# blobcache/glfs

Measured on AMD Instinct MI355X. Metric: GiB/s hashed, device-resident 1 MiB chunks, bigblob write; 1/2/4/8 MI355X, higher is better.
Workload: dtype u32; 1 GPU; bigblob write 64 GiB/GPU @ 1024 KiB blocks, device-resident, ctext to HBM; blob_bytes=68719476736, block_size=1048576, blocks=65536, parallelism=disjoint block ranges x1

## Files before the change

### glfs_amd/csrc/one_classes.h

```cpp
#pragma once
#include <cstddef>
#include <cstdint>
#include <vector>

namespace glfsx {

enum OneClass : uint8_t { kOneSmall = 0, kOneMed = 1, kOneOpen = 2, kOneOpenSalted = 3 };
constexpr int kOneClasses = 4;

struct OneItem {
  bool open;
  bool salted;
  uint64_t len;
};

struct OneLayout {
  uint32_t count[kOneClasses] = {0, 0, 0, 0};
  uint32_t start[kOneClasses] = {0, 0, 0, 0};
  uint64_t max_len[kOneClasses] = {0, 0, 0, 0};
  uint64_t med_bytes = 0;
  std::vector<uint8_t> cls;
  std::vector<uint32_t> slot;
  std::vector<uint64_t> med_off;
};

inline uint64_t one_med_span(uint64_t len) { return (len + 255) & ~uint64_t(255); }

inline OneClass one_class(const OneItem &it, uint64_t small_max) {
  if (it.open) return it.salted ? kOneOpenSalted : kOneOpen;
  return it.len <= small_max ? kOneSmall : kOneMed;
}

inline OneLayout one_layout(const OneItem *items, size_t n, uint64_t small_max) {
  OneLayout L;
  L.cls.resize(n);
  L.slot.resize(n);
  L.med_off.assign(n, 0);
  for (size_t k = 0; k < n; ++k) {
    const OneClass c = one_class(items[k], small_max);
    L.cls[k] = c;
    ++L.count[c];
    if (items[k].len > L.max_len[c]) L.max_len[c] = items[k].len;
  }
  L.start[kOneSmall] = 0;
  L.start[kOneMed] = L.count[kOneSmall];
  L.start[kOneOpen] = 0;
  L.start[kOneOpenSalted] = L.count[kOneOpen];
  uint32_t next[kOneClasses];
  for (int c = 0; c < kOneClasses; ++c) next[c] = L.start[c];
  for (size_t k = 0; k < n; ++k) {
    const uint8_t c = L.cls[k];
    L.slot[k] = next[c]++;
    if (c == kOneMed) {
      L.med_off[k] = L.med_bytes;
      L.med_bytes += one_med_span(items[k].len);
    }
  }
  return L;
}

}
```

### glfs_amd/csrc/one_kernels.h

```cpp


__device__ __forceinline__ uint32_t img_g(uint32_t g) { return g ^ ((g >> 6) & 3u); }

__device__ __forceinline__ void one_chunks(uint32_t &cl, uint32_t &ch, uint32_t img,
                                           uint32_t len, uint32_t ctr0, bool root,
                                           uint32_t kq_lo, uint32_t kq_hi, uint32_t ivq,
                                           uint32_t base, uint32_t q, uint32_t quad,
                                           const uint32_t (&rel)[28]) {
  const uint32_t C = len ? (len + 1023) >> 10 : 1u;
  cl = kq_lo;
  ch = kq_hi;
  if (quad < C) {
    const uint32_t clen = min(len - min(len, quad << 10), 1024u);
    const uint32_t nb = clen ? (clen + 63) >> 6 : 1u;
    uint32_t addr[28];
#pragma unroll
    for (int k = 0; k < 28; ++k) {
      addr[k] = img + (quad << 10) + (rel[k] ^ (16u * (quad & 3u)));
      asm volatile("" : "+v"(addr[k]));
    }
    uint32_t m[4];
#pragma unroll
    for (int k = 0; k < 4; ++k) m[k] = *reinterpret_cast<lds_word>(addr[k]);
#pragma unroll
    for (int b = 0; b < 16; ++b) {
      if (uint32_t(b) < nb) {
        const uint32_t blen = min(clen - min(clen, 64u * b), 64u);
        uint32_t fl = base;
        if (b == 0) fl |= kChunkStart;
        if (uint32_t(b) + 1 == nb) {
          fl |= kChunkEnd;
          if (root && C == 1) fl |= kRoot;
        }
        const uint32_t dq = qsel(q, ctr0 + quad, 0u, blen, fl);
        uint32_t ab[28], nxt[4];
#pragma unroll
        for (int k = 0; k < 28; ++k) ab[k] = addr[k] + 64u * b;
        const uint32_t nb_off = uint32_t(b) + 1 < nb ? 64u * (b + 1) : 64u * b;
#pragma unroll
        for (int k = 0; k < 4; ++k) nxt[k] = addr[k] + nb_off;
        quad_compress_m<true>(cl, ch, ivq, dq, ab, m, nxt);
      }
    }
  }
}

__device__ __forceinline__ void one_tree(uint32_t &cl, uint32_t &ch, uint32_t count,
                                         bool root, uint32_t ts, uint32_t *passbuf,
                                         uint32_t kq_lo, uint32_t kq_hi, uint32_t ivq,
                                         uint32_t base, uint32_t q, uint32_t quad,
                                         const uint32_t (&rel)[28]) {
  while (count > 1) {
    const uint32_t half = count >> 1, odd = count & 1u;
    __syncthreads();
    if (quad < count) {
      if (odd && quad == count - 1) {
        passbuf[q] = cl;
        passbuf[4 + q] = ch;
      } else {
        const uint32_t sa = ts + ((quad >> 1) << 6) + ((quad & 1u) << 5) + 4u * q;
        *reinterpret_cast<__attribute__((address_space(3))) uint32_t *>(sa) = cl;
        *reinterpret_cast<__attribute__((address_space(3))) uint32_t *>(sa + 16u) = ch;
      }
    }
    __syncthreads();
    if (quad < half) {
      const uint32_t fl = base | kParent | ((root && count == 2) ? kRoot : 0u);
      cl = kq_lo;
      ch = kq_hi;
      const uint32_t dq = qsel(q, 0u, 0u, 64u, fl);
      uint32_t addr[28];
#pragma unroll
      for (int k = 0; k < 28; ++k) addr[k] = ts + (quad << 6) + rel[k];
      quad_compress(cl, ch, ivq, dq, addr);
    } else if (odd && quad == half) {
      cl = passbuf[q];
      ch = passbuf[4 + q];
    }
    count = half + odd;
  }
}

__device__ __forceinline__ void one_hash(uint32_t &cl, uint32_t &ch, uint32_t img,
                                         uint32_t ts, uint32_t *passbuf,
                                         uint32_t len, const uint32_t (&key)[8],
                                         uint32_t base, uint32_t q, uint32_t quad,
                                         const uint32_t (&rel)[28], uint32_t ctr0 = 0,
                                         bool root = true) {
  const uint32_t kq_lo = qsel(q, key[0], key[1], key[2], key[3]);
  const uint32_t kq_hi = qsel(q, key[4], key[5], key[6], key[7]);
  const uint32_t ivq = qsel(q, kIV[0], kIV[1], kIV[2], kIV[3]);
  one_chunks(cl, ch, img, len, ctr0, root, kq_lo, kq_hi, ivq, base, q, quad, rel);
  const uint32_t C = len ? (len + 1023) >> 10 : 1u;
  one_tree(cl, ch, C, root, ts, passbuf, kq_lo, kq_hi, ivq, base, q, quad, rel);
}

template <int LANES, int IT = 16>
__device__ __forceinline__ void one_stage(uint4 *img_u4, const uint8_t *src, uint32_t len,
                                          uint32_t present, uint8_t *dcopy) {
  const uint32_t padded = len ? (len + 63) & ~63u : 64u;
  const uint32_t have = min(len, present);
  uint4 v[IT];
#pragma unroll
  for (int i = 0; i < IT; ++i) {
    const uint32_t p = (threadIdx.x + uint32_t(i) * LANES) * 16u;
    v[i] = make_uint4(0, 0, 0, 0);
    if (p + 16u <= have) v[i] = *reinterpret_cast<const uint4 *>(src + p);
  }
#pragma unroll
  for (int i = 0; i < IT; ++i) {
    const uint32_t p = (threadIdx.x + uint32_t(i) * LANES) * 16u;
    if (p < padded) {
      if (p < have && p + 16u > have) {
        uint32_t w[4] = {0, 0, 0, 0};
        for (uint32_t k = 0; p + k < have; ++k) w[k >> 2] |= uint32_t(src[p + k]) << (8 * (k & 3));
        v[i] = make_uint4(w[0], w[1], w[2], w[3]);
      }
      img_u4[img_g(p >> 4)] = v[i];
      if (dcopy) *reinterpret_cast<uint4 *>(dcopy + p) = v[i];
    }
  }
}

template <int LANES>
__device__ __forceinline__ void one_xor(uint4 *img_u4, uint32_t len, const uint32_t (&dek)[8],
                                        uint32_t kb0) {
  const uint32_t nks = (len + 63) >> 6;
  for (uint32_t kb = threadIdx.x; kb < nks; kb += LANES) {
    uint32_t x[16];
    chacha_block<0>(x, dek, kb0 + kb);
    const uint32_t avail = min(len - kb * 64u, 64u);
    if (avail < 64) mask_tail(x, avail);
#pragma unroll
    for (int i = 0; i < 4; ++i) {
      uint4 v = img_u4[img_g(kb * 4 + i)];
      v.x ^= x[4 * i];
      v.y ^= x[4 * i + 1];
      v.z ^= x[4 * i + 2];
      v.w ^= x[4 * i + 3];
      img_u4[img_g(kb * 4 + i)] = v;
    }
  }
}

template <int LANES>
__device__ __forceinline__ void one_store(const uint4 *img_u4, uint8_t *dst, uint32_t len) {
  for (uint32_t p = threadIdx.x * 16u; p < len; p += LANES * 16u) {
    const uint4 v = img_u4[img_g(p >> 4)];
    if (p + 16u <= len) {
      *reinterpret_cast<uint4 *>(dst + p) = v;
    } else {
      const uint32_t w[4] = {v.x, v.y, v.z, v.w};
      for (uint32_t i = 0; p + i < len; ++i) dst[p + i] = uint8_t(w[i >> 2] >> (8 * (i & 3)));
    }
  }
}

template <class D>
__device__ __forceinline__ const D *one_desc(D *s, const D *g) {
  constexpr uint32_t kW = sizeof(D) / 4;
  static_assert(sizeof(D) % 4 == 0 && kW <= 64, "wave 0 stages the descriptor");
  if (threadIdx.x < kW)
    reinterpret_cast<uint32_t *>(s)[threadIdx.x] =
        reinterpret_cast<const uint32_t *>(g)[threadIdx.x];
  __syncthreads();
  return s;
}

template <class D>
__device__ __forceinline__ void one_signal(const D *dp) {
  asm volatile("s_waitcnt vmcnt(0)" ::: "memory");
  __syncthreads();
  if (threadIdx.x == 0 && dp->flag)
    __hip_atomic_store(dp->flag, dp->seq, __ATOMIC_RELEASE, __HIP_MEMORY_SCOPE_SYSTEM);
}

#if GLFSX_ONE_TIMING
__device__ unsigned long long g_one_t[16];
#define ONE_T(i)                                                                        \
  do {                                                                                  \
    if (blockIdx.x == 0 && threadIdx.x == 0)                                            \
      __hip_atomic_fetch_add(&g_one_t[i],                                               \
                             (unsigned long long)(__builtin_amdgcn_s_memrealtime() - t0), \
                             __ATOMIC_RELAXED, __HIP_MEMORY_SCOPE_AGENT);               \
  } while (0)
#else
#define ONE_T(i) \
  do {           \
  } while (0)
#endif

template <int QUADS, bool V>
__device__ __forceinline__ void one_run(const OneDesc *g) {
#if GLFSX_ONE_TIMING
  const uint64_t t0 = __builtin_amdgcn_s_memrealtime(), c0 = __builtin_amdgcn_s_memtime();
#endif
  __shared__ uint4 img_u4[QUADS * 64];
  __shared__ uint4 ts_u4[QUADS / 2 * 4];
  __shared__ uint32_t passbuf[8];
  __shared__ uint32_t s_dek[8];
  constexpr int kLanes = QUADS * 4;
  const OneDesc *dp;
  if constexpr (V) {
    dp = g;
  } else {
    __shared__ OneDesc s_desc;
    dp = one_desc(&s_desc, g + blockIdx.x);
  }
  const uint32_t len = dp->len;
  const uint32_t tid = threadIdx.x, q = tid & 3u, quad = tid >> 2;
  const uint32_t img = lds_offset(img_u4), ts = lds_offset(ts_u4);
  ONE_T(0);
  one_stage<kLanes>(img_u4, dp->src, len, dp->present, nullptr);
  uint32_t rel[28];
  quad_addrs(rel, 0u, q);
  __syncthreads();
  ONE_T(1);
  uint32_t key[8];
#pragma unroll
  for (int i = 0; i < 8; ++i) key[i] = dp->salt[i];
  uint32_t cl, ch;
#if GLFSX_ONE_TIMING
  {
    const uint32_t kq_lo = qsel(q, key[0], key[1], key[2], key[3]);
    const uint32_t kq_hi = qsel(q, key[4], key[5], key[6], key[7]);
    const uint32_t ivq = qsel(q, kIV[0], kIV[1], kIV[2], kIV[3]);
    one_chunks(cl, ch, img, len, 0u, true, kq_lo, kq_hi, ivq, kKeyed, q, quad, rel);
    ONE_T(6);
    one_tree(cl, ch, len ? (len + 1023) >> 10 : 1u, true, ts, passbuf, kq_lo, kq_hi, ivq,
             kKeyed, q, quad, rel);
  }
#else
  one_hash(cl, ch, img, ts, passbuf, len, key, kKeyed, q, quad, rel);
#endif
  if (quad == 0) {
    s_dek[q] = cl;
    s_dek[4 + q] = ch;
  }
  __syncthreads();
  ONE_T(2);
  uint32_t dek[8];
#pragma unroll
  for (int i = 0; i < 8; ++i) dek[i] = s_dek[i];
  one_xor<kLanes>(img_u4, len, dek, 0u);
  __syncthreads();
  ONE_T(3);
  if (dp->ctext) one_store<kLanes>(img_u4, dp->ctext, len);
  uint32_t ckey[8];
#pragma unroll
  for (int i = 0; i < 8; ++i) ckey[i] = dp->cid_key[i];
#if GLFSX_ONE_TIMING
  {
    const uint32_t cb = dp->cid_keyed ? kKeyed : 0u;
    const uint32_t kq_lo = qsel(q, ckey[0], ckey[1], ckey[2], ckey[3]);
    const uint32_t kq_hi = qsel(q, ckey[4], ckey[5], ckey[6], ckey[7]);
    const uint32_t ivq = qsel(q, kIV[0], kIV[1], kIV[2], kIV[3]);
    one_chunks(cl, ch, img, len, 0u, true, kq_lo, kq_hi, ivq, cb, q, quad, rel);
    ONE_T(7);
    one_tree(cl, ch, len ? (len + 1023) >> 10 : 1u, true, ts, passbuf, kq_lo, kq_hi, ivq, cb,
             q, quad, rel);
  }
#else
  one_hash(cl, ch, img, ts, passbuf, len, ckey, dp->cid_keyed ? kKeyed : 0u, q, quad, rel);
#endif
  if (quad == 0) {
    uint32_t *r = reinterpret_cast<uint32_t *>(dp->ref);
    r[q] = cl;
    r[4 + q] = ch;
    r[8 + q] = dek[q];
    r[12 + q] = dek[4 + q];
  }
  ONE_T(4);
  one_signal(dp);
  ONE_T(5);
#if GLFSX_ONE_TIMING
  if (blockIdx.x == 0 && threadIdx.x == 0) {
    const uint64_t c1 = __builtin_amdgcn_s_memtime(), t1 = __builtin_amdgcn_s_memrealtime();
    __hip_atomic_fetch_add(&g_one_t[13], (unsigned long long)(c1 - c0), __ATOMIC_RELAXED,
                           __HIP_MEMORY_SCOPE_AGENT);
    __hip_atomic_fetch_add(&g_one_t[14], (unsigned long long)(t1 - t0), __ATOMIC_RELAXED,
                           __HIP_MEMORY_SCOPE_AGENT);
    __hip_atomic_fetch_add(&g_one_t[15], 1ull, __ATOMIC_RELAXED, __HIP_MEMORY_SCOPE_AGENT);
  }
#endif
}

template <int QUADS>
__global__ __launch_bounds__(QUADS * 4) void k_one(const OneDesc *descs) {
  one_run<QUADS, false>(descs);
}

template <int QUADS>
__global__ __launch_bounds__(QUADS * 4) void k_one_v(const OneDesc d) {
  one_run<QUADS, true>(&d);
}

__device__ __forceinline__ void med_publish_merge(uint32_t &cl, uint32_t &ch, const OneDesc *dp,
                                                  uint32_t sidx, uint32_t W, uint32_t ts,
                                                  uint32_t *passbuf, uint32_t *flag,
                                                  const uint32_t (&key)[8], uint32_t base,
                                                  uint32_t q, uint32_t quad,
                                                  const uint32_t (&rel)[28], bool *last) {
  const uint32_t tid = threadIdx.x;
  if (quad == 0) {
    __hip_atomic_store(dp->cvs + sidx * 8 + q, cl, __ATOMIC_RELAXED, __HIP_MEMORY_SCOPE_AGENT);
    __hip_atomic_store(dp->cvs + sidx * 8 + 4 + q, ch, __ATOMIC_RELAXED,
                       __HIP_MEMORY_SCOPE_AGENT);
  }
  *last = arrive_last(dp->cnt, W, tid, flag);
  if (!*last) return;
// ... 130 lines not shown
```

### glfs_amd/csrc/post_kernels.hip

```cpp
#include "kernels.h"

#include <algorithm>
#include <atomic>
#include <cstdlib>
#include <cstring>
#include <mutex>
#include <type_traits>
#include <utility>

#include "device_common.h"
#include "launch_plan.h"
#include "stream_scratch.h"

namespace glfsx {
namespace {

#include "b3_arx.h"
#include "pass_kernels.h"
#include "quad_kernels.h"
#include "one_kernels.h"
#include "one_open_kernels.h"
#include "small_kernels.h"
#include "ragged_kernels.h"
#include "read_kernels.h"
#include "open_kernels.h"
#include "ragged_open_kernels.h"


std::atomic<uint32_t> g_latency_wgs{512}, g_split_target{2048u};
Knobs knobs() {
  return {g_split_target.load(std::memory_order_relaxed),
          g_latency_wgs.load(std::memory_order_relaxed)};
}

LaunchLog &g_launch_log = *new LaunchLog();
LaunchLog &g_aux_log = *new LaunchLog();

template <const auto &Gs, class F, size_t... I>
hipError_t with_g(uint32_t g, F &&f, std::index_sequence<I...>) {
  hipError_t e = hipErrorInvalidValue;
  (void)(... || (g == uint32_t(Gs[I]) && ((e = f(std::integral_constant<int, Gs[I]>{})), true)));
  return e;
}
template <const auto &Gs, class F>
hipError_t with_g(uint32_t g, F &&f) {
  return with_g<Gs>(g, f, std::make_index_sequence<std::size(Gs)>{});
}

template <int G, bool CHACHA, bool ALIGNED, int A>
bool try_pass(const LaunchRec &r, const KArgs &a, hipStream_t s) {
  if constexpr (pass_form_ok(G, CHACHA, ALIGNED, A)) {
    if (r.chacha == CHACHA && r.aligned == ALIGNED && r.form == A) {
      hipLaunchKernelGGL((k_pass<G, CHACHA, ALIGNED, A>), dim3(r.grid), dim3(256), 0, s, a);
      return true;
    }
  }
  return false;
}
template <int G, bool CHACHA>
bool try_pass_g(const LaunchRec &r, const KArgs &a, hipStream_t s) {
  return try_pass<G, CHACHA, true, 0>(r, a, s) || try_pass<G, CHACHA, true, 1>(r, a, s) ||
         try_pass<G, CHACHA, true, 2>(r, a, s) || try_pass<G, CHACHA, false, 2>(r, a, s);
}

// ... 422 lines not shown
  for (int i = 0; i < 3; ++i) totals[i] = __atomic_load_n(tot + i, __ATOMIC_RELAXED);
  if (totals[0] == 0) return hipSuccess;
  e = get(0, 4 * size_t(cv_words) * (totals[0] + totals[1]));
  a.gcv = a.cvs + cv_words * totals[0];
  return e;
}

template <bool CHACHA>
static hipError_t launch_rag_pass(RArgs a, const uint64_t tot[3], hipStream_t s) {
  a.total = tot[0];
  const GridForm p = rag_chunk_plan(tot[0], knobs().latency_wgs);
  if (p.form == 0)
    hipLaunchKernelGGL((k_rag_chunk<CHACHA, 0>), dim3(p.grid), dim3(256), 0, s, a);
  else
    hipLaunchKernelGGL((k_rag_chunk<CHACHA, 2>), dim3(p.grid), dim3(256), 0, s, a);
  hipError_t e = hipGetLastError();
  auto merge = [&](auto k, uint64_t total) {
    a.total = total;
    hipLaunchKernelGGL(k, dim3(capped_grid(total, 1u << 20)), dim3(256), 0, s, a);
    return hipGetLastError();
  };
  if (e == hipSuccess && tot[1]) e = merge(k_rag_merge_a, tot[1]);
  if (e == hipSuccess && tot[2]) e = merge(k_rag_merge_b, tot[2]);
  return e;
}

hipError_t launch_post_ragged(const RaggedJob &job, hipStream_t s) {
  if (job.n == 0) return hipSuccess;
  if (job.hi > kMaxRaggedLen) return hipErrorInvalidValue;
  RArgs a{};
  a.src = job.src;
  a.ctext = job.ctext;
  a.offs = job.offs;
  a.lens = job.lens;
  a.n = job.n;
  a.lo = job.lo;
  a.hi = job.hi;
  a.refs = job.refs;
  uint64_t totals[3];
  hipError_t e = rag_plan<false>(a, &ScratchSlot::rag, 8, nullptr, 0u, totals, s);
  if (e != hipSuccess || totals[0] == 0) return e;
  for (int i = 0; i < 8; ++i) a.key[i] = job.salt[i];
  a.base = kKeyed;
  a.out_off = 32;
  e = launch_rag_pass<false>(a, totals, s);
  if (e != hipSuccess) return e;
  for (int i = 0; i < 8; ++i) a.key[i] = job.cid_key[i];
  a.base = job.cid_keyed ? kKeyed : 0u;
  a.out_off = 0;
  return launch_rag_pass<true>(a, totals, s);
}

#if GLFSX_ONE_TIMING
extern "C" int glfsx_debug_one_timing(int reset, uint64_t out[16]) {
  if (hipMemcpyFromSymbol(out, HIP_SYMBOL(g_one_t), 16 * sizeof(uint64_t), 0,
                          hipMemcpyDeviceToHost) != hipSuccess)
    return -1;
  if (!reset) return 0;
  const unsigned long long z[16] = {};
  return hipMemcpyToSymbol(HIP_SYMBOL(g_one_t), z, sizeof z, 0, hipMemcpyHostToDevice) ==
                 hipSuccess ? 0 : -1;
}
#endif

size_t pass_log(int reset, uint32_t *out, size_t cap) {
  if (!g_launch_log.on()) g_launch_log.enable();
  return g_launch_log.read(reset != 0, out, cap);
}

size_t aux_log(int reset, uint32_t *out, size_t cap) {
  if (!g_aux_log.on()) g_aux_log.enable();
  return g_aux_log.read(reset != 0, out, cap);
}

hipError_t clock_probe(int reset, uint64_t out[2]) {
  g_clk_on.store(true, std::memory_order_relaxed);
  unsigned long long v[2] = {0, 0};
  hipError_t e = hipMemcpyFromSymbol(v, HIP_SYMBOL(g_clk), sizeof v, 0, hipMemcpyDeviceToHost);
  if (e != hipSuccess) return e;
  if (out) {
    out[0] = v[0];
    out[1] = v[1];
  }
  if (!reset) return hipSuccess;
  const unsigned long long z[2] = {0, 0};
  return hipMemcpyToSymbol(HIP_SYMBOL(g_clk), z, sizeof z, 0, hipMemcpyHostToDevice);
}

#if GLFSX_WGTIME
hipError_t debug_wgtime(uint64_t *out) {
  return hipMemcpyFromSymbol(out, HIP_SYMBOL(g_wgtime), sizeof(g_wgtime), 0,
                             hipMemcpyDeviceToHost);
}
#endif

template <class K, class A>
static hipError_t med_launch(K dek, K cid, uint32_t n, uint64_t len, const A &a, hipStream_t s) {
  if (len > kMaxMedLen || len <= kMaxOneLen) return hipErrorInvalidValue;
  const uint32_t wmax = uint32_t((len + 65535) >> 16);
  hipLaunchKernelGGL(dek, dim3(n * wmax), dim3(256), 0, s, a, wmax);
  hipError_t e = hipGetLastError();
  if (e != hipSuccess) return e;
  hipLaunchKernelGGL(cid, dim3(n * wmax), dim3(256), 0, s, a, wmax);
  return hipGetLastError();
}
hipError_t launch_med(const OneDesc *descs, uint32_t n, uint64_t max_len, hipStream_t s) {
  return n ? med_launch(k_med_dek, k_med_cid, n, max_len, descs, s) : hipSuccess;
}
hipError_t launch_med_v(const OneDesc &d, hipStream_t s) {
  return med_launch(k_med_dek_v, k_med_cid_v, 1, d.len, d, s);
}

template <class K, class A>
static hipError_t one_launch(K k16, K k64, uint32_t n, uint64_t len, const A &a, hipStream_t s) {
  if (len > kMaxOneLen) return hipErrorInvalidValue;
  if (len <= 16 * 1024)
    hipLaunchKernelGGL(k16, dim3(n), dim3(64), 0, s, a);
  else
    hipLaunchKernelGGL(k64, dim3(n), dim3(256), 0, s, a);
  return hipGetLastError();
}
hipError_t launch_one(const OneDesc *descs, uint32_t n, uint64_t max_len, hipStream_t s) {
  return n ? one_launch(k_one<16>, k_one<64>, n, max_len, descs, s) : hipSuccess;
}
hipError_t launch_one_v(const OneDesc &d, hipStream_t s) {
  return one_launch(k_one_v<16>, k_one_v<64>, 1, d.len, d, s);
}

template <class K, class A>
static hipError_t one_open_launch(K k16s, K k64s, K k16, K k64, uint32_t n, uint64_t len,
                                  bool salted, const A &a, hipStream_t s) {
  if (len > kMaxOneLen) return hipErrorInvalidValue;
  const bool small = len <= 16 * 1024;
  const K k = salted ? (small ? k16s : k64s) : (small ? k16 : k64);
  hipLaunchKernelGGL(k, dim3(n), dim3((small ? 16 : 64) * (salted ? 8 : 4)), 0, s, a);
  return hipGetLastError();
}
hipError_t launch_one_open(const OneOpenDesc *descs, uint32_t n, uint64_t max_len, bool salted,
                           hipStream_t s) {
  if (n == 0) return hipSuccess;
  return one_open_launch(k_one_open<16, true>, k_one_open<64, true>, k_one_open<16, false>,
                         k_one_open<64, false>, n, max_len, salted, descs, s);
}
hipError_t launch_one_open_v(const OneOpenDesc &d, bool salted, hipStream_t s) {
  return one_open_launch(k_one_open_v<16, true>, k_one_open_v<64, true>, k_one_open_v<16, false>,
                         k_one_open_v<64, false>, 1, d.len, salted, d, s);
}

hipError_t launch_decrypt(const uint8_t *ctext, uint8_t *ptext, uint64_t n, uint64_t bs,
                          uint64_t last_len, const uint8_t *refs, hipStream_t s) {
  return decrypt_with(ctext, ptext, n, bs, last_len, refs, knobs().latency_wgs, s);
}

hipError_t launch_chacha_xor(const uint32_t k[8], const uint8_t *src,
                             uint8_t *dst, uint64_t n, hipStream_t s) {
  if (n == 0) return hipSuccess;
  KArgs a{};
  a.src = src;
  a.ctext = dst;
  a.msg_len = n;
  for (int i = 0; i < 8; ++i) a.key[i] = k[i];
  const uint32_t grid = capped_grid((((n + 63) >> 6) + 255) / 256, 65536);
  hipLaunchKernelGGL(k_chacha_xor, dim3(grid), dim3(256), 0, s, a);
  return hipGetLastError();
}


static std::atomic<int> g_open_route{0};
int set_open_route(int route) {
// ... 131 lines not shown
```

### glfs_amd/csrc/quad_kernels.h

```cpp

#define QCOL0_ASM                                                               \
  "v_add_u32 %0, %1, %4\n"                                                      \
  "v_xor_b32 %3, %3, %0\n"                                                      \
  "v_alignbit_b32 %3, %3, %3, 16\n"                                             \
  "v_add_u32 %2, %2, %3\n"                                                      \
  "v_xor_b32 %1, %1, %2\n"                                                      \
  "v_alignbit_b32 %1, %1, %1, 12\n"
#define QCOL_ASM                                                                \
  "s_nop 0\n"                                                                   \
  "v_add_u32_dpp %0, %1, %4 quad_perm:[3,0,1,2] row_mask:0xf bank_mask:0xf\n"   \
  "v_xor_b32_dpp %3, %3, %0 quad_perm:[1,2,3,0] row_mask:0xf bank_mask:0xf\n"   \
  "v_alignbit_b32 %3, %3, %3, 16\n"                                             \
  "v_add_u32_dpp %2, %2, %3 quad_perm:[2,3,0,1] row_mask:0xf bank_mask:0xf\n"   \
  "v_xor_b32_dpp %1, %1, %2 quad_perm:[3,0,1,2] row_mask:0xf bank_mask:0xf\n"   \
  "v_alignbit_b32 %1, %1, %1, 12\n"
#define QREST_ASM                                                               \
  "v_add3_u32 %0, %0, %1, %5\n"                                                 \
  "v_xor_b32 %3, %3, %0\n"                                                      \
  "v_alignbit_b32 %3, %3, %3, 8\n"                                              \
  "v_add_u32 %2, %2, %3\n"                                                      \
  "v_xor_b32 %1, %1, %2\n"                                                      \
  "v_alignbit_b32 %1, %1, %1, 7\n"                                              \
  "v_add_u32 %4, %0, %6\n"                                                      \
  "s_nop 0\n"                                                                   \
  "v_add_u32_dpp %0, %1, %4 quad_perm:[1,2,3,0] row_mask:0xf bank_mask:0xf\n"   \
  "v_xor_b32_dpp %3, %3, %0 quad_perm:[3,0,1,2] row_mask:0xf bank_mask:0xf\n"   \
  "v_alignbit_b32 %3, %3, %3, 16\n"                                             \
  "v_add_u32_dpp %2, %2, %3 quad_perm:[2,3,0,1] row_mask:0xf bank_mask:0xf\n"   \
  "v_xor_b32_dpp %1, %1, %2 quad_perm:[1,2,3,0] row_mask:0xf bank_mask:0xf\n"   \
  "v_alignbit_b32 %1, %1, %1, 12\n"                                             \
  "v_add3_u32 %0, %0, %1, %7\n"                                                 \
  "v_xor_b32 %3, %3, %0\n"                                                      \
  "v_alignbit_b32 %3, %3, %3, 8\n"                                              \
  "v_add_u32 %2, %2, %3\n"                                                      \
  "v_xor_b32 %1, %1, %2\n"                                                      \
  "v_alignbit_b32 %1, %1, %1, 7\n"

typedef const __attribute__((address_space(3))) uint32_t *lds_word;
template <bool PF>
__device__ __forceinline__ void quad_compress_m(uint32_t &a, uint32_t &b, uint32_t c,
                                                uint32_t d, const uint32_t (&addr)[28],
                                                uint32_t (&m)[4], const uint32_t *nxt) {
#pragma unroll
  for (int r = 0; r < 7; ++r) {
    uint32_t n[4] = {0, 0, 0, 0};
    if (r < 6) {
#pragma unroll
      for (int k = 0; k < 4; ++k) n[k] = *reinterpret_cast<lds_word>(addr[4 * r + 4 + k]);
    } else if (PF) {
#pragma unroll
      for (int k = 0; k < 4; ++k) n[k] = *reinterpret_cast<lds_word>(nxt[k]);
    }
// ... 40 lines not shown
                              kSched.s[r][kk[k] + 4], kSched.s[r][kk[k] + 6]);
      addr[4 * r + k] = slot + 4u * (w ^ x);
    }
  }
}

__device__ __forceinline__ void tree_reduce_q(uint32_t *lds, uint32_t k, uint32_t t,
                              const uint32_t (&key)[8], uint32_t base, bool root,
                              uint32_t (&p)[8]) {
  const uint32_t q = t & 3u, quad = t >> 2;
  const uint32_t kq_lo = qsel(q, key[0], key[1], key[2], key[3]);
  const uint32_t kq_hi = qsel(q, key[4], key[5], key[6], key[7]);
  const uint32_t ivq = qsel(q, kIV[0], kIV[1], kIV[2], kIV[3]);
  uint32_t rel[28];
  quad_addrs(rel, lds_offset(lds), q);
  while (k > 1) {
    const uint32_t half = k >> 1, odd = k & 1u;
    const uint32_t fl = base | kParent | ((root && k == 2) ? kRoot : 0u);
    const uint32_t dq = qsel(q, 0u, 0u, 64u, fl);
    uint32_t rl[2] = {0, 0}, rh[2] = {0, 0};
#pragma unroll
    for (uint32_t r = 0; r < 2; ++r) {
      const uint32_t i = quad + 64u * r;
      if (i < half) {
        uint32_t addr[28];
#pragma unroll
        for (int x = 0; x < 28; ++x) addr[x] = rel[x] + 64u * i;
        uint32_t cl = kq_lo, ch = kq_hi;
        quad_compress(cl, ch, ivq, dq, addr);
        rl[r] = cl;
        rh[r] = ch;
      }
    }
    const uint32_t ov = (odd && t < 8) ? lds[(k - 1) * 8 + t] : 0u;
    __syncthreads();
#pragma unroll
    for (uint32_t r = 0; r < 2; ++r) {
      const uint32_t i = quad + 64u * r;
      if (i < half) {
        lds[i * 8 + q] = rl[r];
        lds[i * 8 + 4 + q] = rh[r];
      }
    }
    if (odd && t < 8) lds[half * 8 + t] = ov;
    __syncthreads();
    k = half + odd;
  }
  if (t == 0) {
#pragma unroll
    for (int i = 0; i < 8; ++i) p[i] = lds[i];
  }
}

template <int QPW>
__global__ __launch_bounds__(QPW * 4) void k_quad(KArgs a) {
  constexpr bool kTwo = QPW == 64;
  __shared__ uint4 slots[QPW * (kTwo ? 8 : 4)];
  __shared__ uint32_t passbuf[8];
  const uint32_t tid = threadIdx.x, q = tid & 3u, quad = tid >> 2;
  const uint64_t j = blockIdx.x >> a.split_log2;
  const uint32_t sidx = blockIdx.x & ((1u << a.split_log2) - 1u);
  const uint64_t len = (j + 1 == a.n) ? a.last_len : a.msg_len;
  constexpr uint64_t kSpan = uint64_t(QPW) << 10;
  const uint64_t c0b = uint64_t(sidx) * kSpan;
  if (sidx != 0 && c0b >= len) return;
  const bool whole = len <= kSpan;
  const uint64_t mylen = min(len - c0b, kSpan);
  const uint32_t cnt = mylen ? uint32_t((mylen + 1023) >> 10) : 1u;
  const uint8_t *msg = a.src + j * a.stride + c0b;
  const uint32_t slot = lds_offset(slots + quad * 4);
  const uint32_t kq_lo = qsel(q, a.key[0], a.key[1], a.key[2], a.key[3]);
  const uint32_t kq_hi = qsel(q, a.key[4], a.key[5], a.key[6], a.key[7]);
  const uint32_t ivq = qsel(q, kIV[0], kIV[1], kIV[2], kIV[3]);
  uint32_t addr[28];
  quad_addrs(addr, slot, q);
  uint32_t cl = kq_lo, ch = kq_hi;
  if (quad < cnt) {
    const uint64_t coff = uint64_t(quad) << 10;
    const uint32_t clen = uint32_t(min<uint64_t>(mylen - coff, 1024));
    const uint32_t nb = clen ? (clen + 63) >> 6 : 1u;
    const uint32_t ctr = sidx * uint32_t(QPW) + quad;
    const uint8_t *cp = msg + coff + 16u * q;
    uint4 blk[16];
#pragma unroll
    for (int b = 0; b < 16; ++b) {
      blk[b] = make_uint4(0, 0, 0, 0);
      const int32_t avail = int32_t(clen) - 64 * b - 16 * int32_t(q);
      if (avail >= 16) {
        blk[b] = *reinterpret_cast<const uint4 *>(cp + 64 * b);
      } else if (avail > 0) {
        uint32_t w[4] = {0, 0, 0, 0};
        for (int i = 0; i < avail; ++i) w[i >> 2] |= uint32_t(cp[64 * b + i]) << (8 * (i & 3));
        blk[b] = make_uint4(w[0], w[1], w[2], w[3]);
      }
    }
    const uint32_t x = kTwo ? 4u * ((quad >> 1) & 3u) : 0u;
    const uint32_t gq = 16u * (q ^ (x >> 2));
    constexpr uint32_t kB = kTwo ? QPW * 64u : 0u;
    uint32_t caddr[28];
    if constexpr (kTwo) {
      quad_addrs(caddr, slot, q, x);
#pragma unroll
      for (int k = 0; k < 28; ++k) asm volatile("" : "+v"(caddr[k]));
    }
    uint32_t m[4];
    if constexpr (kTwo) {
      *reinterpret_cast<lds_u32x4 *>(slot + gq) =
          u32x4{blk[0].x, blk[0].y, blk[0].z, blk[0].w};
      asm volatile("" ::: "memory");
#pragma unroll
      for (int k = 0; k < 4; ++k) m[k] = *reinterpret_cast<lds_word>(caddr[k]);
    }
#pragma unroll
    for (int b = 0; b < 16; ++b) {
      if (uint32_t(b) < nb) {
        const bool more = uint32_t(b) + 1 < nb;
        if constexpr (kTwo) {
          if (b + 1 < 16 && more)
            *reinterpret_cast<lds_u32x4 *>(slot + kB * ((b + 1) & 1) + gq) =
                u32x4{blk[(b + 1) & 15].x, blk[(b + 1) & 15].y, blk[(b + 1) & 15].z,
                      blk[(b + 1) & 15].w};
        } else {
          *reinterpret_cast<lds_u32x4 *>(slot + gq) =
              u32x4{blk[b].x, blk[b].y, blk[b].z, blk[b].w};
        }
        asm volatile("" ::: "memory");
        const uint32_t blen = min(clen - min(clen, 64u * b), 64u);
        uint32_t fl = a.base;
        if (b == 0) fl |= kChunkStart;
        if (uint32_t(b) + 1 == nb) {
          fl |= kChunkEnd;
          if (whole && cnt == 1) fl |= kRoot;
        }
        const uint32_t dq = qsel(q, ctr, 0u, blen, fl);
        if constexpr (kTwo) {
          uint32_t ab[28], nxt[4];
#pragma unroll
          for (int k = 0; k < 28; ++k) ab[k] = caddr[k] + kB * (b & 1);
          const uint32_t noff = more ? kB * ((b + 1) & 1) : kB * (b & 1);
#pragma unroll
          for (int k = 0; k < 4; ++k) nxt[k] = caddr[k] + noff;
          quad_compress_m<true>(cl, ch, ivq, dq, ab, m, nxt);
        } else {
          quad_compress(cl, ch, ivq, dq, addr);
        }
        asm volatile("" ::: "memory");
      }
    }
  }
  uint32_t count = cnt;
  while (count > 1) {
    const uint32_t half = count >> 1, odd = count & 1u;
    __syncthreads();
    if (quad < count) {
      if (odd && quad == count - 1) {
        passbuf[q] = cl;
        passbuf[4 + q] = ch;
      } else {
        uint32_t *ps = reinterpret_cast<uint32_t *>(slots + (quad >> 1) * 4);
        ps[(quad & 1u) * 8 + q] = cl;
        ps[(quad & 1u) * 8 + 4 + q] = ch;
      }
    }
    __syncthreads();
    if (quad < half) {
      const uint32_t fl = a.base | kParent | ((whole && count == 2) ? kRoot : 0u);
      cl = kq_lo;
      ch = kq_hi;
      const uint32_t dq = qsel(q, 0u, 0u, 64u, fl);
      quad_compress(cl, ch, ivq, dq, addr);
    } else if (odd && quad == half) {
      cl = passbuf[q];
      ch = passbuf[4 + q];
    }
    count = half + odd;
  }
  uint32_t *const out = reinterpret_cast<uint32_t *>(
      a.refs + (j / a.ref_bf) * a.ref_stride + (j % a.ref_bf) * 64 + a.out_off);
  if (whole) {
    if (quad == 0) {
      out[q] = cl;
      out[4 + q] = ch;
    }
    return;
  }
  const uint64_t wbase = j << a.split_log2;
  if (tid < 64) {
    uint32_t w[8];
#pragma unroll
    for (int k = 0; k < 4; ++k) {
      w[k] = __builtin_amdgcn_readlane(cl, k);
      w[4 + k] = __builtin_amdgcn_readlane(ch, k);
    }
    if (tid == 0) publish_cv(a.scratch + (wbase + sidx) * 8, w);
  }
  const uint32_t W = uint32_t((len + kSpan - 1) / kSpan);
  __shared__ uint32_t s_flag;
  if (!arrive_last(a.cnt + j, W, tid, &s_flag)) return;
  if (quad < W) {
    cl = load_cv_word(a.scratch + (wbase + quad) * 8 + q);
    ch = load_cv_word(a.scratch + (wbase + quad) * 8 + 4 + q);
  }
  count = W;
  while (count > 1) {
    const uint32_t half = count >> 1, odd = count & 1u;
    __syncthreads();
    if (quad < count) {
      if (odd && quad == count - 1) {
        passbuf[q] = cl;
        passbuf[4 + q] = ch;
      } else {
        uint32_t *ps = reinterpret_cast<uint32_t *>(slots + (quad >> 1) * 4);
        ps[(quad & 1u) * 8 + q] = cl;
        ps[(quad & 1u) * 8 + 4 + q] = ch;
      }
    }
    __syncthreads();
    if (quad < half) {
      const uint32_t fl = a.base | kParent | (count == 2 ? kRoot : 0u);
      cl = kq_lo;
      ch = kq_hi;
      const uint32_t dq = qsel(q, 0u, 0u, 64u, fl);
      quad_compress(cl, ch, ivq, dq, addr);
    } else if (odd && quad == half) {
      cl = passbuf[q];
      ch = passbuf[4 + q];
    }
    count = half + odd;
  }
  if (quad == 0) {
    out[q] = cl;
    out[4 + q] = ch;
    if (q == 0) a.cnt[j] = 0;
  }
}
```

Baseline: 968.6 GiB/s.

## Specialize full-chunk BLAKE3 path, add quad-parallel ChaCha XOR, tighten one-kernel threshold

Adds a FULL template specialization of the per-quad chunk compression. When a wave-wide ballot shows every chunk is a full 1 KiB, it uses precomputed flags and unconditional loads and skips the prefetch on the last block. It also adds a quad-cooperative ChaCha implementation using DPP lane permutes for the XOR stage, and lowers the single-wave launch threshold for the one-shot kernel from 16 KiB to 1 KiB. It further expands the debug timing counters. The goal is to remove per-block branch and flag arithmetic and to spread keystream work across more lanes, at the cost of larger code and more register pressure from the template duplication.

```diff
diff --git a/glfs_amd/csrc/one_classes.h b/glfs_amd/csrc/one_classes.h
--- a/glfs_amd/csrc/one_classes.h
+++ b/glfs_amd/csrc/one_classes.h
@@ -25,6 +25,8 @@
 };
 
 inline uint64_t one_med_span(uint64_t len) { return (len + 255) & ~uint64_t(255); }
+
+constexpr uint64_t kOneWaveMaxLen = 1024;
 
 inline OneClass one_class(const OneItem &it, uint64_t small_max) {
   if (it.open) return it.salted ? kOneOpenSalted : kOneOpen;
diff --git a/glfs_amd/csrc/one_kernels.h b/glfs_amd/csrc/one_kernels.h
--- a/glfs_amd/csrc/one_kernels.h
+++ b/glfs_amd/csrc/one_kernels.h
@@ -1,17 +1,28 @@
 
 
 __device__ __forceinline__ uint32_t img_g(uint32_t g) { return g ^ ((g >> 6) & 3u); }
+
+#if GLFSX_ONE_TIMING
+#define ONE_C_ARGS , uint64_t c0 = 0, int cslot = -1
+#define ONE_C_BLOCK(b) \
+  if (cslot >= 0) ONE_C(cslot + (b))
+#else
+#define ONE_C_ARGS
+#define ONE_C_BLOCK(b)
+#endif
 
 __device__ __forceinline__ void one_chunks(uint32_t &cl, uint32_t &ch, uint32_t img,
                                            uint32_t len, uint32_t ctr0, bool root,
                                            uint32_t kq_lo, uint32_t kq_hi, uint32_t ivq,
                                            uint32_t base, uint32_t q, uint32_t quad,
-                                           const uint32_t (&rel)[28]) {
+                                           const uint32_t (&rel)[28] ONE_C_ARGS) {
   const uint32_t C = len ? (len + 1023) >> 10 : 1u;
   cl = kq_lo;
   ch = kq_hi;
-  if (quad < C) {
-    const uint32_t clen = min(len - min(len, quad << 10), 1024u);
+  const bool mine = quad < C;
+  const uint32_t clen = mine ? min(len - min(len, quad << 10), 1024u) : 0u;
+  const bool full = __builtin_amdgcn_ballot_w64(mine && clen != 1024u) == 0;
+  if (mine) {
     const uint32_t nb = clen ? (clen + 63) >> 6 : 1u;
     uint32_t addr[28];
 #pragma unroll
@@ -22,6 +33,27 @@
     uint32_t m[4];
 #pragma unroll
     for (int k = 0; k < 4; ++k) m[k] = *reinterpret_cast<lds_word>(addr[k]);
+    if (full) {
+      const uint32_t lane3 = q == 3 ? ~0u : 0u;
+      const uint32_t dq = qsel(q, ctr0 + quad, 0u, 64u, base);
+      const uint32_t end = kChunkEnd | ((root && C == 1) ? kRoot : 0u);
+#pragma unroll
+      for (int b = 0; b < 16; ++b) {
+        uint32_t ab[28], nxt[4];
+#pragma unroll
+        for (int k = 0; k < 28; ++k) ab[k] = addr[k] + 64u * b;
+#pragma unroll
+        for (int k = 0; k < 4; ++k) nxt[k] = addr[k] + 64u * (b + 1);
+        if (b == 0)
+          quad_compress_m<true>(cl, ch, ivq, dq | (kChunkStart & lane3), ab, m, nxt);
+        else if (b < 15)
+          quad_compress_m<true>(cl, ch, ivq, dq, ab, m, nxt);
+        else
+          quad_compress_m<false>(cl, ch, ivq, dq | (end & lane3), ab, m, nullptr);
+        ONE_C_BLOCK(b);
+      }
+      return;
+    }
 #pragma unroll
     for (int b = 0; b < 16; ++b) {
       if (uint32_t(b) < nb) {
@@ -41,6 +73,7 @@
         for (int k = 0; k < 4; ++k) nxt[k] = addr[k] + nb_off;
         quad_compress_m<true>(cl, ch, ivq, dq, ab, m, nxt);
       }
+      ONE_C_BLOCK(b);
     }
   }
 }
@@ -122,10 +155,82 @@
   }
 }
 
+#define CQ_REST                                                                 \
+  "v_xor_b32 %3, %3, %0\n"                                                      \
+  "v_alignbit_b32 %3, %3, %3, 24\n"                                             \
+  "v_add_u32 %2, %2, %3\n"                                                      \
+  "v_xor_b32 %1, %1, %2\n"                                                      \
+  "v_alignbit_b32 %1, %1, %1, 25\n"
+#define CQ_COL0                                                                 \
+  "v_add_u32 %0, %0, %1\n"                                                      \
+  "v_xor_b32 %3, %3, %0\n"                                                      \
+  "v_alignbit_b32 %3, %3, %3, 16\n"                                             \
+  "v_add_u32 %2, %2, %3\n"                                                      \
+  "v_xor_b32 %1, %1, %2\n"                                                      \
+  "v_alignbit_b32 %1, %1, %1, 20\n"                                             \
+  "v_add_u32 %0, %0, %1\n" CQ_REST
+#define CQ_STEP(P1, P2, P3)                                                     \
+  "s_nop 1\n"                                                                   \
+  "v_add_u32_dpp %0, %1, %0 quad_perm:" P1 " row_mask:0xf bank_mask:0xf\n"      \
+  "v_xor_b32_dpp %3, %3, %0 quad_perm:" P3 " row_mask:0xf bank_mask:0xf\n"      \
+  "v_alignbit_b32 %3, %3, %3, 16\n"                                             \
+  "v_add_u32_dpp %2, %2, %3 quad_perm:" P2 " row_mask:0xf bank_mask:0xf\n"      \
+  "v_xor_b32_dpp %1, %1, %2 quad_perm:" P1 " row_mask:0xf bank_mask:0xf\n"      \
+  "v_alignbit_b32 %1, %1, %1, 20\n"                                             \
+  "v_add_u32 %0, %0, %1\n" CQ_REST
+#define CQ_DIAG CQ_STEP("[1,2,3,0]", "[2,3,0,1]", "[3,0,1,2]")
+#define CQ_COL CQ_STEP("[3,0,1,2]", "[2,3,0,1]", "[1,2,3,0]")
+
+__device__ __forceinline__ void chacha_quad(uint32_t &a, uint32_t &b, uint32_t &c, uint32_t &d,
+                                            const uint32_t (&k)[8], uint32_t ctr, uint32_t q) {
+  const uint32_t a0 = qsel(q, 0x61707865u, 0x3320646eu, 0x79622d32u, 0x6b206574u);
+  const uint32_t b0 = qsel(q, k[0], k[1], k[2], k[3]);
+  const uint32_t c0 = qsel(q, k[4], k[5], k[6], k[7]);
+  const uint32_t d0 = q == 0 ? ctr : 0u;
+  a = a0;
+  b = b0;
+  c = c0;
+  d = d0;
+  asm volatile(CQ_COL0 CQ_DIAG : "+v"(a), "+v"(b), "+v"(c), "+v"(d));
+#pragma unroll
+  for (int i = 1; i < 10; ++i)
+    asm volatile(CQ_COL CQ_DIAG : "+v"(a), "+v"(b), "+v"(c), "+v"(d));
+  asm volatile("v_add_u32 %0, %0, %4\n"
+               "v_add_u32_dpp %3, %3, %7 quad_perm:[1,2,3,0] row_mask:0xf bank_mask:0xf\n"
+               "v_add_u32_dpp %2, %2, %6 quad_perm:[2,3,0,1] row_mask:0xf bank_mask:0xf\n"
+               "v_add_u32_dpp %1, %1, %5 quad_perm:[3,0,1,2] row_mask:0xf bank_mask:0xf\n"
+               : "+v"(a), "+v"(b), "+v"(c), "+v"(d)
+               : "v"(a0), "v"(b0), "v"(c0), "v"(d0));
+}
+
 template <int LANES>
 __device__ __forceinline__ void one_xor(uint4 *img_u4, uint32_t len, const uint32_t (&dek)[8],
                                         uint32_t kb0) {
   const uint32_t nks = (len + 63) >> 6;
+  constexpr uint32_t kQuads = LANES / 4;
+  if ((nks + kQuads - 1) / kQuads <= 2u * ((nks + LANES - 1) / LANES)) {
+    const uint32_t q = threadIdx.x & 3u;
+    const uint32_t imgw = lds_offset(img_u4) + 4u * q;
+    for (uint32_t kb = threadIdx.x >> 2; kb < nks; kb += kQuads) {
+      uint32_t wa[4], v[4];
+#pragma unroll
+      for (int i = 0; i < 4; ++i) {
+        wa[i] = imgw + 16u * img_g(kb * 4 + i);
+        v[i] = *reinterpret_cast<lds_word>(wa[i]);
+      }
+      uint32_t x[4];
+      chacha_quad(x[0], x[1], x[2], x[3], dek, kb0 + kb, q);
+      const uint32_t avail = len - kb * 64u;
+#pragma unroll
+      for (int i = 0; i < 4; ++i) {
+        const uint32_t lo = 16u * i + 4u * q;
+        if (avail < lo + 4u)
+          x[i] &= avail <= lo ? 0u : (1u << (8u * (avail - lo))) - 1u;
+        *reinterpret_cast<__attribute__((address_space(3))) uint32_t *>(wa[i]) = v[i] ^ x[i];
+      }
+    }
+    return;
+  }
   for (uint32_t kb = threadIdx.x; kb < nks; kb += LANES) {
     uint32_t x[16];
     chacha_block<0>(x, dek, kb0 + kb);
@@ -176,13 +281,13 @@
 }
 
 #if GLFSX_ONE_TIMING
-__device__ unsigned long long g_one_t[16];
 #define ONE_T(i)                                                                        \
   do {                                                                                  \
     if (blockIdx.x == 0 && threadIdx.x == 0)                                            \
       __hip_atomic_fetch_add(&g_one_t[i],                                               \
                              (unsigned long long)(__builtin_amdgcn_s_memrealtime() - t0), \
                              __ATOMIC_RELAXED, __HIP_MEMORY_SCOPE_AGENT);               \
+    ONE_C(32 + (i));                                                                    \
   } while (0)
 #else
 #define ONE_T(i) \
@@ -225,7 +330,7 @@
     const uint32_t kq_lo = qsel(q, key[0], key[1], key[2], key[3]);
     const uint32_t kq_hi = qsel(q, key[4], key[5], key[6], key[7]);
     const uint32_t ivq = qsel(q, kIV[0], kIV[1], kIV[2], kIV[3]);
-    one_chunks(cl, ch, img, len, 0u, true, kq_lo, kq_hi, ivq, kKeyed, q, quad, rel);
+    one_chunks(cl, ch, img, len, 0u, true, kq_lo, kq_hi, ivq, kKeyed, q, quad, rel, c0, 16);
     ONE_T(6);
     one_tree(cl, ch, len ? (len + 1023) >> 10 : 1u, true, ts, passbuf, kq_lo, kq_hi, ivq,
              kKeyed, q, quad, rel);
@@ -246,6 +351,9 @@
   __syncthreads();
   ONE_T(3);
   if (dp->ctext) one_store<kLanes>(img_u4, dp->ctext, len);
+#if GLFSX_ONE_TIMING
+  ONE_C(56);
+#endif
   uint32_t ckey[8];
 #pragma unroll
   for (int i = 0; i < 8; ++i) ckey[i] = dp->cid_key[i];
@@ -255,7 +363,7 @@
     const uint32_t kq_lo = qsel(q, ckey[0], ckey[1], ckey[2], ckey[3]);
     const uint32_t kq_hi = qsel(q, ckey[4], ckey[5], ckey[6], ckey[7]);
     const uint32_t ivq = qsel(q, kIV[0], kIV[1], kIV[2], kIV[3]);
-    one_chunks(cl, ch, img, len, 0u, true, kq_lo, kq_hi, ivq, cb, q, quad, rel);
+    one_chunks(cl, ch, img, len, 0u, true, kq_lo, kq_hi, ivq, cb, q, quad, rel, c0, 40);
     ONE_T(7);
     one_tree(cl, ch, len ? (len + 1023) >> 10 : 1u, true, ts, passbuf, kq_lo, kq_hi, ivq, cb,
              q, quad, rel);
diff --git a/glfs_amd/csrc/post_kernels.hip b/glfs_amd/csrc/post_kernels.hip
--- a/glfs_amd/csrc/post_kernels.hip
+++ b/glfs_amd/csrc/post_kernels.hip
@@ -10,6 +10,7 @@
 
 #include "device_common.h"
 #include "launch_plan.h"
+#include "one_classes.h"
 #include "stream_scratch.h"
 
 namespace glfsx {
@@ -538,12 +539,12 @@
 }
 
 #if GLFSX_ONE_TIMING
-extern "C" int glfsx_debug_one_timing(int reset, uint64_t out[16]) {
-  if (hipMemcpyFromSymbol(out, HIP_SYMBOL(g_one_t), 16 * sizeof(uint64_t), 0,
+extern "C" int glfsx_debug_one_timing(int reset, uint64_t out[64]) {
+  if (hipMemcpyFromSymbol(out, HIP_SYMBOL(g_one_t), 64 * sizeof(uint64_t), 0,
                           hipMemcpyDeviceToHost) != hipSuccess)
     return -1;
   if (!reset) return 0;
-  const unsigned long long z[16] = {};
+  const unsigned long long z[64] = {};
   return hipMemcpyToSymbol(HIP_SYMBOL(g_one_t), z, sizeof z, 0, hipMemcpyHostToDevice) ==
                  hipSuccess ? 0 : -1;
 }
@@ -600,7 +601,7 @@
 template <class K, class A>
 static hipError_t one_launch(K k16, K k64, uint32_t n, uint64_t len, const A &a, hipStream_t s) {
   if (len > kMaxOneLen) return hipErrorInvalidValue;
-  if (len <= 16 * 1024)
+  if (len <= kOneWaveMaxLen)
     hipLaunchKernelGGL(k16, dim3(n), dim3(64), 0, s, a);
   else
     hipLaunchKernelGGL(k64, dim3(n), dim3(256), 0, s, a);
diff --git a/glfs_amd/csrc/quad_kernels.h b/glfs_amd/csrc/quad_kernels.h
--- a/glfs_amd/csrc/quad_kernels.h
+++ b/glfs_amd/csrc/quad_kernels.h
@@ -1,3 +1,20 @@
+
+#if GLFSX_ONE_TIMING
+__device__ unsigned long long g_one_t[64];
+#define ONE_N(i)                                                                 \
+  do {                                                                           \
+    if (blockIdx.x == 0 && threadIdx.x == 0)                                     \
+      __hip_atomic_fetch_add(&g_one_t[i], 1ull, __ATOMIC_RELAXED,                \
+                             __HIP_MEMORY_SCOPE_AGENT);                          \
+  } while (0)
+#define ONE_C(i)                                                                    \
+  do {                                                                              \
+    if (blockIdx.x == 0 && threadIdx.x == 0)                                        \
+      __hip_atomic_fetch_add(&g_one_t[i],                                           \
+                             (unsigned long long)(__builtin_amdgcn_s_memtime() - c0), \
+                             __ATOMIC_RELAXED, __HIP_MEMORY_SCOPE_AGENT);           \
+  } while (0)
+#endif
 
 #define QCOL0_ASM                                                               \
   "v_add_u32 %0, %1, %4\n"                                                      \
@@ -144,11 +161,105 @@
   }
 }
 
+template <int QPW, bool FULL>
+__device__ __forceinline__ void quad_chunk(uint32_t &cl, uint32_t &ch, const uint8_t *cp,
+                                           uint32_t clen, uint32_t ctr, uint32_t base,
+                                           bool rootable, uint32_t ivq, uint32_t slot,
+                                           uint32_t q, uint32_t quad,
+                                           const uint32_t (&addr)[28]) {
+  constexpr bool kTwo = QPW == 64;
+  const uint32_t nb = FULL ? 16u : clen ? (clen + 63) >> 6 : 1u;
+  uint4 blk[16];
+#pragma unroll
+  for (int b = 0; b < 16; ++b) {
+    blk[b] = make_uint4(0, 0, 0, 0);
+    const int32_t avail = int32_t(clen) - 64 * b - 16 * int32_t(q);
+    if (FULL || avail >= 16) {
+      blk[b] = *reinterpret_cast<const uint4 *>(cp + 64 * b);
+    } else if (avail > 0) {
+      uint32_t w[4] = {0, 0, 0, 0};
+      for (int i = 0; i < avail; ++i) w[i >> 2] |= uint32_t(cp[64 * b + i]) << (8 * (i & 3));
+      blk[b] = make_uint4(w[0], w[1], w[2], w[3]);
+    }
+  }
+  const uint32_t x = kTwo ? 4u * ((quad >> 1) & 3u) : 0u;
+  const uint32_t gq = 16u * (q ^ (x >> 2));
+  constexpr uint32_t kB = kTwo ? QPW * 64u : 0u;
+  uint32_t caddr[28];
+  if constexpr (kTwo) {
+    quad_addrs(caddr, slot, q, x);
+#pragma unroll
+    for (int k = 0; k < 28; ++k) asm volatile("" : "+v"(caddr[k]));
+  }
+  const uint32_t lane3 = q == 3 ? ~0u : 0u, dq_full = qsel(q, ctr, 0u, 64u, base);
+  uint32_t m[4];
+  if constexpr (kTwo) {
+    *reinterpret_cast<lds_u32x4 *>(slot + gq) =
+        u32x4{blk[0].x, blk[0].y, blk[0].z, blk[0].w};
+    asm volatile("" ::: "memory");
+#pragma unroll
+    for (int k = 0; k < 4; ++k) m[k] = *reinterpret_cast<lds_word>(caddr[k]);
+  }
+#pragma unroll
+  for (int b = 0; b < 16; ++b) {
+    if (FULL || uint32_t(b) < nb) {
+      const bool more = FULL ? b + 1 < 16 : uint32_t(b) + 1 < nb;
+      if constexpr (kTwo) {
+        if (b + 1 < 16 && more)
+          *reinterpret_cast<lds_u32x4 *>(slot + kB * ((b + 1) & 1) + gq) =
+              u32x4{blk[(b + 1) & 15].x, blk[(b + 1) & 15].y, blk[(b + 1) & 15].z,
+                    blk[(b + 1) & 15].w};
+      } else {
+        *reinterpret_cast<lds_u32x4 *>(slot + gq) =
+            u32x4{blk[b].x, blk[b].y, blk[b].z, blk[b].w};
+      }
+      asm volatile("" ::: "memory");
+      uint32_t dq;
+      if constexpr (FULL) {
+        const uint32_t fl = (b == 0 ? kChunkStart : 0u) |
+                            (b == 15 ? kChunkEnd | (rootable ? kRoot : 0u) : 0u);
+        dq = dq_full | (fl & lane3);
+      } else {
+        const uint32_t blen = min(clen - min(clen, 64u * b), 64u);
+        uint32_t fl = base;
+        if (b == 0) fl |= kChunkStart;
+        if (uint32_t(b) + 1 == nb) {
+          fl |= kChunkEnd;
+          if (rootable) fl |= kRoot;
+        }
+        dq = qsel(q, ctr, 0u, blen, fl);
+      }
+      if constexpr (kTwo) {
+        uint32_t ab[28], nxt[4];
+#pragma unroll
+        for (int k = 0; k < 28; ++k) ab[k] = caddr[k] + kB * (b & 1);
+        const uint32_t noff = more ? kB * ((b + 1) & 1) : kB * (b & 1);
+#pragma unroll
+        for (int k = 0; k < 4; ++k) nxt[k] = caddr[k] + noff;
+        if (FULL && b == 15)
+          quad_compress_m<false>(cl, ch, ivq, dq, ab, m, nullptr);
+        else
+          quad_compress_m<true>(cl, ch, ivq, dq, ab, m, nxt);
+      } else {
+        quad_compress(cl, ch, ivq, dq, addr);
+      }
+      asm volatile("" ::: "memory");
+    }
+  }
+}
+
 template <int QPW>
 __global__ __launch_bounds__(QPW * 4) void k_quad(KArgs a) {
   constexpr bool kTwo = QPW == 64;
   __shared__ uint4 slots[QPW * (kTwo ? 8 : 4)];
   __shared__ uint32_t passbuf[8];
+#if GLFSX_ONE_TIMING
+  const uint64_t c0 = __builtin_amdgcn_s_memtime();
+#define QUAD_C(i) \
+  if (QPW == 64) ONE_C(i)
+#else
+#define QUAD_C(i)
+#endif
   const uint32_t tid = threadIdx.x, q = tid & 3u, quad = tid >> 2;
   const uint64_t j = blockIdx.x >> a.split_log2;
   const uint32_t sidx = blockIdx.x & ((1u << a.split_log2) - 1u);
@@ -167,79 +278,21 @@
   uint32_t addr[28];
   quad_addrs(addr, slot, q);
   uint32_t cl = kq_lo, ch = kq_hi;
-  if (quad < cnt) {
-    const uint64_t coff = uint64_t(quad) << 10;
-    const uint32_t clen = uint32_t(min<uint64_t>(mylen - coff, 1024));
-    const uint32_t nb = clen ? (clen + 63) >> 6 : 1u;
+  const bool mine = quad < cnt;
+  const uint32_t clen = mine ? uint32_t(min<uint64_t>(mylen - (uint64_t(quad) << 10), 1024)) : 0u;
+  const bool full = kTwo && __builtin_amdgcn_ballot_w64(mine && clen != 1024u) == 0;
+  QUAD_C(57);
+  if (mine) {
     const uint32_t ctr = sidx * uint32_t(QPW) + quad;
-    const uint8_t *cp = msg + coff + 16u * q;
-    uint4 blk[16];
-#pragma unroll
-    for (int b = 0; b < 16; ++b) {
-      blk[b] = make_uint4(0, 0, 0, 0);
-      const int32_t avail = int32_t(clen) - 64 * b - 16 * int32_t(q);
-      if (avail >= 16) {
-        blk[b] = *reinterpret_cast<const uint4 *>(cp + 64 * b);
-      } else if (avail > 0) {
-        uint32_t w[4] = {0, 0, 0, 0};
-        for (int i = 0; i < avail; ++i) w[i >> 2] |= uint32_t(cp[64 * b + i]) << (8 * (i & 3));
-        blk[b] = make_uint4(w[0], w[1], w[2], w[3]);
-      }
-    }
-    const uint32_t x = kTwo ? 4u * ((quad >> 1) & 3u) : 0u;
-    const uint32_t gq = 16u * (q ^ (x >> 2));
-    constexpr uint32_t kB = kTwo ? QPW * 64u : 0u;
-    uint32_t caddr[28];
-    if constexpr (kTwo) {
-      quad_addrs(caddr, slot, q, x);
-#pragma unroll
-      for (int k = 0; k < 28; ++k) asm volatile("" : "+v"(caddr[k]));
-    }
-    uint32_t m[4];
-    if constexpr (kTwo) {
-      *reinterpret_cast<lds_u32x4 *>(slot + gq) =
-          u32x4{blk[0].x, blk[0].y, blk[0].z, blk[0].w};
-      asm volatile("" ::: "memory");
-#pragma unroll
-      for (int k = 0; k < 4; ++k) m[k] = *reinterpret_cast<lds_word>(caddr[k]);
-    }
-#pragma unroll
-    for (int b = 0; b < 16; ++b) {
-      if (uint32_t(b) < nb) {
-        const bool more = uint32_t(b) + 1 < nb;
-        if constexpr (kTwo) {
-          if (b + 1 < 16 && more)
-            *reinterpret_cast<lds_u32x4 *>(slot + kB * ((b + 1) & 1) + gq) =
-                u32x4{blk[(b + 1) & 15].x, blk[(b + 1) & 15].y, blk[(b + 1) & 15].z,
-                      blk[(b + 1) & 15].w};
-        } else {
-          *reinterpret_cast<lds_u32x4 *>(slot + gq) =
-              u32x4{blk[b].x, blk[b].y, blk[b].z, blk[b].w};
-        }
-        asm volatile("" ::: "memory");
-        const uint32_t blen = min(clen - min(clen, 64u * b), 64u);
-        uint32_t fl = a.base;
-        if (b == 0) fl |= kChunkStart;
-        if (uint32_t(b) + 1 == nb) {
-          fl |= kChunkEnd;
-          if (whole && cnt == 1) fl |= kRoot;
-        }
-        const uint32_t dq = qsel(q, ctr, 0u, blen, fl);
-        if constexpr (kTwo) {
-          uint32_t ab[28], nxt[4];
-#pragma unroll
-          for (int k = 0; k < 28; ++k) ab[k] = caddr[k] + kB * (b & 1);
-          const uint32_t noff = more ? kB * ((b + 1) & 1) : kB * (b & 1);
-#pragma unroll
-          for (int k = 0; k < 4; ++k) nxt[k] = caddr[k] + noff;
-          quad_compress_m<true>(cl, ch, ivq, dq, ab, m, nxt);
-        } else {
-          quad_compress(cl, ch, ivq, dq, addr);
-        }
-        asm volatile("" ::: "memory");
-      }
-    }
-  }
+    const uint8_t *cp = msg + (uint64_t(quad) << 10) + 16u * q;
+    if (full)
+      quad_chunk<QPW, true>(cl, ch, cp, clen, ctr, a.base, whole && cnt == 1, ivq, slot, q, quad,
+                            addr);
+    else
+      quad_chunk<QPW, false>(cl, ch, cp, clen, ctr, a.base, whole && cnt == 1, ivq, slot, q, quad,
+                             addr);
+  }
+  QUAD_C(58);
   uint32_t count = cnt;
   while (count > 1) {
     const uint32_t half = count >> 1, odd = count & 1u;
@@ -267,6 +320,7 @@
     }
     count = half + odd;
   }
+  QUAD_C(59);
   uint32_t *const out = reinterpret_cast<uint32_t *>(
       a.refs + (j / a.ref_bf) * a.ref_stride + (j % a.ref_bf) * 64 + a.out_off);
   if (whole) {
@@ -274,6 +328,10 @@
       out[q] = cl;
       out[4 + q] = ch;
     }
+    QUAD_C(60);
+#if GLFSX_ONE_TIMING
+    if (QPW == 64) ONE_N(63);
+#endif
     return;
   }
   const uint64_t wbase = j << a.split_log2;
@@ -288,7 +346,14 @@
   }
   const uint32_t W = uint32_t((len + kSpan - 1) / kSpan);
   __shared__ uint32_t s_flag;
+  QUAD_C(60);
+#if GLFSX_ONE_TIMING
+  if (QPW == 64) ONE_N(63);
+#endif
   if (!arrive_last(a.cnt + j, W, tid, &s_flag)) return;
+#if GLFSX_ONE_TIMING
+  const uint64_t c1 = __builtin_amdgcn_s_memtime();
+#endif
   if (quad < W) {
     cl = load_cv_word(a.scratch + (wbase + quad) * 8 + q);
     ch = load_cv_word(a.scratch + (wbase + quad) * 8 + 4 + q);
@@ -325,4 +390,12 @@
     out[4 + q] = ch;
     if (q == 0) a.cnt[j] = 0;
   }
-}
+#if GLFSX_ONE_TIMING
+  if (QPW == 64 && tid == 0) {
+    __hip_atomic_fetch_add(&g_one_t[61], (unsigned long long)(__builtin_amdgcn_s_memtime() - c1),
+                           __ATOMIC_RELAXED, __HIP_MEMORY_SCOPE_AGENT);
+    __hip_atomic_fetch_add(&g_one_t[62], 1ull, __ATOMIC_RELAXED, __HIP_MEMORY_SCOPE_AGENT);
+  }
+#endif
+#undef QUAD_C
+}
```

Result: no change. 970.5 GiB/s, median of 2 (+0.2%).
